# QEDProtocol/city-rollup

Hardware: AMD Instinct MI355X
Metric: ms/NTT at 2^20 Goldilocks (commit-shaped step: 135-column 2^20-row NTT + Poseidon Merkle cap) (lower is better)
Workload: dtype u64 (Goldilocks mod 2^64-2^32+1; the Poseidon MDS layers are evaluated exactly on 32-bit limbs held in f64); 1 GPU; configs[1]: 2^20-row x 135-column trace, forward NTT per column (natural->bit-reversed) + Poseidon Merkle cap height 4; log_n=20, columns=135, cap_height=4

## Files before the change

### city-rollup_amd/cityprover/__init__.py

```python
import ctypes
import os

import numpy as np

from . import build as _build

P = 0xFFFFFFFF00000001
NTT_INVERSE, NTT_BITREV_OUT, NTT_COSET, NTT_BITREV_IN = 1, 2, 4, 8

_u64p = ctypes.POINTER(ctypes.c_uint64)
_vp = ctypes.c_void_p

ABI = {
    "cp_abi_version": (ctypes.c_int, []),
    "cp_device_count": (ctypes.c_int, []),
    "cp_fault_inject": (ctypes.c_int, [ctypes.c_int, ctypes.c_long]),
    "cp_ctx_create": (_vp, [ctypes.c_int]),
    "cp_ctx_destroy": (None, [_vp]),
    "cp_ctx_set_lanes": (ctypes.c_int, [_vp, ctypes.c_int]),
    "cp_ctx_set_device_transcript": (ctypes.c_int, [_vp, ctypes.c_int]),
    "cp_ctx_set_option": (ctypes.c_int, [_vp, ctypes.c_char_p, ctypes.c_long]),
    "cp_last_error": (ctypes.c_char_p, [_vp]),
    "cp_dev_alloc": (ctypes.c_int, [_vp, ctypes.c_size_t, ctypes.POINTER(_vp)]),
    "cp_dev_free": (ctypes.c_int, [_vp, _vp]),
    "cp_host_alloc": (ctypes.c_int, [_vp, ctypes.c_size_t, ctypes.POINTER(_vp)]),
    "cp_host_free": (ctypes.c_int, [_vp, _vp]),
    "cp_h2d": (ctypes.c_int, [_vp, _vp, _vp, ctypes.c_size_t]),
    "cp_d2h": (ctypes.c_int, [_vp, _vp, _vp, ctypes.c_size_t]),
    "cp_d2d": (ctypes.c_int, [_vp, _vp, _vp, ctypes.c_size_t]),
    "cp_sync": (ctypes.c_int, [_vp]),
    "cp_event_create": (ctypes.c_int, [_vp, ctypes.POINTER(_vp)]),
    "cp_event_destroy": (ctypes.c_int, [_vp, _vp]),
    "cp_event_record": (ctypes.c_int, [_vp, _vp]),
    "cp_event_elapsed_ms": (ctypes.c_int, [_vp, _vp, _vp, ctypes.POINTER(ctypes.c_float)]),
    "cp_profile_begin": (ctypes.c_int, [_vp]),
    "cp_profile_end": (ctypes.c_int, [_vp, ctypes.c_char_p, ctypes.c_size_t]),
    "cp_ntt_dev": (ctypes.c_int, [_vp, _vp, ctypes.c_int, ctypes.c_size_t, ctypes.c_size_t,
                                  ctypes.c_uint, ctypes.c_uint64]),
    "cp_ntt": (ctypes.c_int, [_vp, _u64p, ctypes.c_int, ctypes.c_size_t, ctypes.c_uint,
                              ctypes.c_uint64]),
    "cp_lde_dev": (ctypes.c_int, [_vp, _vp, ctypes.c_size_t, ctypes.c_int, ctypes.c_int,
                                  ctypes.c_size_t, ctypes.c_uint64, ctypes.c_uint, _vp,
                                  ctypes.c_size_t]),
    "cp_poseidon_permute_dev": (ctypes.c_int, [_vp, _vp, ctypes.c_size_t]),
    "cp_field_mul": (ctypes.c_int, [_vp, _u64p, _u64p, _u64p, ctypes.c_size_t]),
    "cp_field_mul2": (ctypes.c_int, [_vp, _u64p, _u64p, _u64p, _u64p, _u64p, _u64p, ctypes.c_size_t]),
    "cp_poseidon_permute": (ctypes.c_int, [_vp, _u64p, ctypes.c_size_t]),
    "cp_hash_no_pad": (ctypes.c_int, [_vp, _u64p, ctypes.c_size_t, ctypes.c_size_t, _u64p]),
    "cp_two_to_one": (ctypes.c_int, [_vp, _u64p, _u64p, ctypes.c_size_t, _u64p]),
    "cp_merkle_cols_dev": (ctypes.c_int, [_vp, _vp, ctypes.c_size_t, ctypes.c_size_t,
                                          ctypes.c_size_t, ctypes.c_int, _vp, _vp]),
    "cp_merkle_cap": (ctypes.c_int, [_vp, _u64p, ctypes.c_size_t, ctypes.c_size_t, ctypes.c_int,
                                     _u64p]),
    "cp_commit_dev": (ctypes.c_int, [_vp, _vp, ctypes.c_size_t, ctypes.c_int, ctypes.c_int,
                                     ctypes.c_int, _vp, _vp, _vp, _vp]),
    "cp_commit_batch_dev": (ctypes.c_int, [_vp, _vp, ctypes.c_size_t, ctypes.c_size_t, ctypes.c_int,
                                           ctypes.c_int, ctypes.c_int, _vp, _vp, _vp, _vp]),
}


class CityProverError(RuntimeError):
    pass


_lib = None


def load_library(build_if_missing=True):
    global _lib
    if _lib is not None:
        return _lib
    so = _build.SO
    if not os.path.exists(so):
        if not build_if_missing:
            raise CityProverError(f"{so} not built; run __graft_entry__.build()")
        _build.build()
    lib = ctypes.CDLL(so)
    for name, (res, args) in ABI.items():
        f = getattr(lib, name)
# ... 166 lines not shown
        self._check(self.lib.cp_ntt(self.ctx, _ptr(a), log_n, batch, flags, shift))
        return a

    def intt(self, a, flags=0, shift=0):
        return self.ntt(a, flags | NTT_INVERSE, shift)

    def lde(self, coeffs, rate_bits, shift=7, bitrev=False):
        c = _as_u64(coeffs)
        c2 = c.reshape(1, -1) if c.ndim == 1 else c
        k, n = c2.shape
        log_n = int(n).bit_length() - 1
        din, dout = self.to_device(c2), self.alloc(k * (n << rate_bits))
        try:
            self.lde_dev(din.ptr, log_n, rate_bits, k, dout.ptr, shift, NTT_BITREV_OUT if bitrev else 0)
            out = dout.download().reshape(k, n << rate_bits)
        finally:
            din.free()
            dout.free()
        return out[0] if c.ndim == 1 else out

    def field_mul(self, a, b):
        x, y = _as_u64(a).ravel().copy(), _as_u64(b).ravel().copy()
        assert x.size == y.size
        out = np.zeros(x.size, np.uint64)
        self._check(self.lib.cp_field_mul(self.ctx, _ptr(x), _ptr(y), _ptr(out), x.size))
        return out

    def field_mul2(self, a, b, c, d):
        v = [_as_u64(x).ravel().copy() for x in (a, b, c, d)]
        assert all(x.size == v[0].size for x in v)
        out_ab, out_cd = np.zeros(v[0].size, np.uint64), np.zeros(v[0].size, np.uint64)
        self._check(self.lib.cp_field_mul2(self.ctx, _ptr(v[0]), _ptr(v[1]), _ptr(v[2]), _ptr(v[3]), _ptr(out_ab), _ptr(out_cd), v[0].size))
        return out_ab, out_cd

    def poseidon_permute(self, states):
        s = _as_u64(states).copy()
        assert s.size % 12 == 0
        self._check(self.lib.cp_poseidon_permute(self.ctx, _ptr(s), s.size // 12))
        return s

    def hash_no_pad(self, inputs):
        x = _as_u64(inputs)
        x2 = x.reshape(1, -1) if x.ndim == 1 else x
        out = np.zeros((x2.shape[0], 4), np.uint64)
        self._check(self.lib.cp_hash_no_pad(self.ctx, _ptr(x2), x2.shape[0], x2.shape[1], _ptr(out)))
        return out[0] if x.ndim == 1 else out

    def two_to_one(self, left, right):
        l, r = _as_u64(left), _as_u64(right)
        l2, r2 = l.reshape(-1, 4), r.reshape(-1, 4)
        out = np.zeros_like(l2)
        self._check(self.lib.cp_two_to_one(self.ctx, _ptr(l2), _ptr(r2), l2.shape[0], _ptr(out)))
        return out.reshape(l.shape)

    def merkle_cap(self, rows, cap_height):
        rows = _as_u64(rows)
        n, k = rows.shape
        cap = np.zeros((1 << cap_height, 4), np.uint64)
        self._check(self.lib.cp_merkle_cap(self.ctx, _ptr(rows), n, k, cap_height, _ptr(cap)))
        return cap

    def merkle_cols(self, cols, cap_height, want_digests=False):
        cols = _as_u64(cols)
        k, n = cols.shape
        dc, dcap = self.to_device(cols), self.alloc(4 << cap_height)
        nd = 2 * n - (2 << cap_height)
# ... 1455 lines not shown
```

### city-rollup_amd/csrc/cityprover.hip

```cpp
#include "core.h"
#include "merkle.h"
#include "ntt.h"
#include "ntt16.h"
#include "poseidon.h"
#include "poseidon_coop.h"

namespace {

int get_pow_table(cp_ctx *ctx, uint64_t base, const uint64_t **out) {
  auto it = ctx->pow_tables.find(base);
  if (it != ctx->pow_tables.end()) {
    *out = it->second.get<uint64_t>();
    return CP_OK;
  }
  std::vector<uint64_t> h(3 * ntt::PT_SIZE);
  uint64_t b = base;
  for (int lvl = 0; lvl < 3; lvl++) {
    uint64_t acc = 1;
    for (int j = 0; j < ntt::PT_SIZE; j++) {
      h[lvl * ntt::PT_SIZE + j] = acc;
      acc = gl::mul(acc, b);
    }
    b = acc;
  }
// ... 700 lines not shown
  return cp_d2h(ctx, out_host, o, bytes);
} CP_CATCH(ctx)

__global__ __launch_bounds__(256) void k_field_mul2(const uint64_t *__restrict__ a, const uint64_t *__restrict__ b,
                                                    const uint64_t *__restrict__ c, const uint64_t *__restrict__ d,
                                                    uint64_t *__restrict__ out_ab, uint64_t *__restrict__ out_cd, size_t n) {
  const size_t i = (size_t)blockIdx.x * 256 + threadIdx.x;
  if (i < n) {
    uint64_t r0, r1;
    gl::mul_lazy2(a[i], b[i], c[i], d[i], r0, r1);
    out_ab[i] = gl::canon(r0);
    out_cd[i] = gl::canon(r1);
  }
}

int cp_field_mul2(cp_ctx *ctx, const uint64_t *a_host, const uint64_t *b_host, const uint64_t *c_host, const uint64_t *d_host,
                  uint64_t *out_ab_host, uint64_t *out_cd_host, size_t count) try {
  CHECK_CTX(ctx);
  if (count == 0) return CP_OK;
  if (!a_host || !b_host || !c_host || !d_host || !out_ab_host || !out_cd_host) return set_error(ctx, CP_ERR_INVALID_ARG, "NULL pointer");
  if (count > ((size_t)1 << 27)) return set_error(ctx, CP_ERR_INVALID_ARG, "count too large");
  const size_t bytes = count * sizeof(uint64_t);
  CP_TRY(ensure_scratch(ctx, 6 * bytes));
  uint64_t *a = ctx->scratch.get<uint64_t>(), *b = a + count, *c = b + count, *d = c + count, *o0 = d + count, *o1 = o0 + count;
  CP_TRY(cp_h2d(ctx, a, a_host, bytes));
  CP_TRY(cp_h2d(ctx, b, b_host, bytes));
  CP_TRY(cp_h2d(ctx, c, c_host, bytes));
  CP_TRY(cp_h2d(ctx, d, d_host, bytes));
  LAUNCH(ctx, "field_mul2", k_field_mul2, dim3(blocks_for(count, 256)), dim3(256), a, b, c, d, o0, o1, count);
  CP_TRY(cp_d2h(ctx, out_ab_host, o0, bytes));
  return cp_d2h(ctx, out_cd_host, o1, bytes);
} CP_CATCH(ctx)


int cp_poseidon_permute_dev(cp_ctx *ctx, uint64_t *states, size_t count) try {
  CHECK_CTX(ctx);
  if (count == 0) return CP_OK;
  if (!states) return set_error(ctx, CP_ERR_INVALID_ARG, "states is NULL");
  LAUNCH(ctx, "poseidon_permute", merkle::k_permute, dim3(blocks_for(count, merkle::THREADS)),
         dim3(merkle::THREADS), states, count);
  return CP_OK;
} CP_CATCH(ctx)

int cp_poseidon_permute(cp_ctx *ctx, uint64_t *states_host, size_t count) try {
  CHECK_CTX(ctx);
  if (count == 0) return CP_OK;
  if (!states_host) return set_error(ctx, CP_ERR_INVALID_ARG, "states is NULL");
  size_t bytes = count * 12 * sizeof(uint64_t);
  CP_TRY(ensure_scratch(ctx, bytes));
  CP_TRY(cp_h2d(ctx, ctx->scratch.get(), states_host, bytes));
  CP_TRY(cp_poseidon_permute_dev(ctx, ctx->scratch.get<uint64_t>(), count));
  return cp_d2h(ctx, states_host, ctx->scratch.get(), bytes);
} CP_CATCH(ctx)

int cp_hash_no_pad(cp_ctx *ctx, const uint64_t *in_host, size_t count, size_t len,
                   uint64_t *digests_host) try {
  CHECK_CTX(ctx);
  if (count == 0) return CP_OK;
  if (!digests_host || (!in_host && len)) return set_error(ctx, CP_ERR_INVALID_ARG, "NULL pointer");
  if (len > (1u << 30)) return set_error(ctx, CP_ERR_INVALID_ARG, "len too large");
  size_t in_bytes = count * len * sizeof(uint64_t), out_bytes = count * 32;
  size_t in_al = (in_bytes + 255) & ~(size_t)255;
  CP_TRY(ensure_scratch(ctx, in_al + out_bytes));
  uint64_t *din = ctx->scratch.get<uint64_t>(), *dout = (uint64_t *)(ctx->scratch.get<char>() + in_al);
  if (in_bytes) CP_TRY(cp_h2d(ctx, din, in_host, in_bytes));
  LAUNCH(ctx, "leaf_hash_rows", merkle::k_leaf_hash_rows, dim3(blocks_for(count, merkle::THREADS)),
// ... 111 lines not shown
```

### city-rollup_amd/csrc/gl.h

```cpp
#pragma once
#include <hip/hip_runtime.h>
#include <stdint.h>

#define GL_HD __host__ __device__ __forceinline__
#if defined(__HIP_DEVICE_COMPILE__) && !defined(GL_PORTABLE)
#define GL_DEVICE_ASM 1
#else
#define GL_DEVICE_ASM 0
#endif

namespace gl {

constexpr uint64_t P = 0xFFFFFFFF00000001ULL;
constexpr uint64_t EPS = 0xFFFFFFFFULL;

GL_HD uint64_t canon(uint64_t x) { return x + (x >= P ? EPS : 0); }

GL_HD uint32_t lo32(uint64_t x) { return (uint32_t)x; }
GL_HD uint32_t hi32(uint64_t x) { return (uint32_t)(x >> 32); }
GL_HD uint64_t pack(uint32_t lo, uint32_t hi) { return ((uint64_t)hi << 32) | lo; }

typedef unsigned __int128 u128;

GL_HD uint64_t sub(uint64_t a, uint64_t b) {
// ... 131 lines not shown
  asm("s_nop 1\n\t"
      "v_subb_co_u32_e64 %0, %4, %7, %8, %10\n\t"
      "v_subb_co_u32_e64 %2, %5, %11, %12, %14\n\t"
      "s_nop 0\n\t"
      "v_subbrev_co_u32_e64 %1, %4, 0, %9, %4\n\t"
      "v_subbrev_co_u32_e64 %3, %5, 0, %13, %5\n\t"
      "s_or_b64 %6, %4, %5"
      : "=&v"(tlA), "=&v"(thA), "=&v"(tlB), "=&v"(thB), "=&s"(bA), "=&s"(bB), "=&s"(bm)
      : "v"(lo32(loA)), "v"(hi32(hiA)), "v"(hi32(loA)), "s"(cyA), "v"(lo32(loB)), "v"(hi32(hiB)), "v"(hi32(loB)), "s"(cyB)
      : "scc");
  uint64_t tA = pack(tlA, thA), tB = pack(tlB, thB);
  if (__builtin_expect(bm != 0, 0)) {
    uint32_t nA, nB;
    asm volatile("s_nop 1\n\tv_cndmask_b32 %0, 0, -1, %2\n\tv_cndmask_b32 %1, 0, -1, %3" : "=&v"(nA), "=v"(nB) : "s"(bA), "s"(bB));
    tA -= nA;
    tB -= nB;
  }
  uint64_t fA, fB, cA, cB, cD;
  uint32_t mA, nB;
  asm("v_mad_u64_u32 %0, %1, %8, -1, %9\n\t"
      "v_mad_u64_u32 %3, %4, %10, -1, %11\n\t"
      "s_nop 0\n\t"
      "v_cndmask_b32 %2, 0, -1, %1\n\t"
      "v_cndmask_b32 %5, 0, 1, %4\n\t"
      "v_mad_u64_u32 %6, %7, %5, -1, %3"
      : "=&v"(fA), "=&s"(cA), "=&v"(mA), "=&v"(fB), "=&s"(cB), "=&v"(nB), "=&v"(r1), "=&s"(cD)
      : "v"(lo32(hiA)), "v"(tA), "v"(lo32(hiB)), "v"(tB));
  r0 = fA + mA;
#else
  r0 = mul_lazy(a0, b0);
  r1 = mul_lazy(a1, b1);
#endif
}
GL_HD uint64_t mul(uint64_t a, uint64_t b) {
  uint64_t lo, hi;
  carry_t cy;
  mul_wide_cy(a, b, lo, hi, cy);
  return reduce128(lo, hi, cy);
}
GL_HD uint64_t sqr(uint64_t a) { return mul(a, a); }
GL_HD uint64_t mul_add_lazy(uint64_t a, uint64_t b, uint64_t c) {
  uint64_t lo, hi;
  carry_t cy;
  mul_wide_cy(a, b, lo, hi, cy);
  lo += c;
  hi += lo < c;
  return reduce128_lazy(lo, hi, cy);
}

GL_HD uint64_t pow7(uint64_t x) {
  uint64_t x2 = sqr(x), x4 = sqr(x2), x3 = mul(x, x2);
  return mul(x3, x4);
}

GL_HD uint64_t pow(uint64_t b, uint64_t e) {
  uint64_t r = 1;
  while (e) {
    if (e & 1) r = mul(r, b);
    b = sqr(b);
    e >>= 1;
  }
  return r;
}
GL_HD uint64_t inv(uint64_t a) { return pow(a, P - 2); }

struct Ext {
// ... 12 lines not shown
```

### city-rollup_amd/csrc/ntt16.h

```cpp
#pragma once
#include <type_traits>

#include "gl.h"
#include "ntt.h"

namespace ntt16 {

template <int K>
GL_HD uint64_t mul_pow2(uint64_t x) {
  static_assert(K >= 0 && K < 96, "shift out of range");
  if constexpr (K == 0) {
    return x;
  } else if constexpr (K < 64) {
    return gl::reduce128(x << K, x >> (64 - K));
  } else {
    constexpr int J = K - 64;
    uint64_t y0 = J ? (x << J) : x;
    uint64_t y1 = J ? (x >> (64 - J)) : 0;
    uint64_t t = gl::reduce128(0, y0);
    return gl::sub(t, y1 << 32);
  }
}

template <bool INV, int E>
GL_HD uint64_t diff_times_w16(uint64_t u, uint64_t v) {
  constexpr int SH = ((INV ? 36 : 156) * (E & 15)) % 192;
  constexpr bool NEG = SH >= 96;
  constexpr int K = SH % 96;
  uint64_t d = NEG ? gl::sub(v, u) : gl::sub(u, v);
  return mul_pow2<K>(d);
}

template <bool INV, int B, bool UNIT_T>
GL_HD void stage(uint64_t (&x)[16], uint64_t T) {
#pragma unroll
  for (int m = 0; m < 16; m++) {
    if (m & (1 << B)) continue;
    const int i = m & ((1 << B) - 1);
    uint64_t u = x[m], v = x[m + (1 << B)];
    x[m] = gl::add(u, v);
    uint64_t d;
    switch (i << (3 - B)) {
      case 0: d = diff_times_w16<INV, 0>(u, v); break;
      case 1: d = diff_times_w16<INV, 1>(u, v); break;
      case 2: d = diff_times_w16<INV, 2>(u, v); break;
      case 3: d = diff_times_w16<INV, 3>(u, v); break;
      case 4: d = diff_times_w16<INV, 4>(u, v); break;
      case 5: d = diff_times_w16<INV, 5>(u, v); break;
      case 6: d = diff_times_w16<INV, 6>(u, v); break;
      default: d = diff_times_w16<INV, 7>(u, v); break;
    }
    x[m + (1 << B)] = UNIT_T ? d : gl::mul(d, T);
  }
}

template <bool INV, int NSTAGES, bool UNIT_T>
GL_HD void round16(uint64_t (&x)[16], uint64_t T3) {
#if defined(NTT16_STAGE_TWIDDLES)
  uint64_t T2 = UNIT_T ? 1 : gl::sqr(T3);
  stage<INV, 3, UNIT_T>(x, T3);
  if constexpr (NSTAGES >= 2) {
    stage<INV, 2, UNIT_T>(x, T2);
  }
  if constexpr (NSTAGES >= 3) {
    uint64_t T1 = UNIT_T ? 1 : gl::sqr(T2);
    stage<INV, 1, UNIT_T>(x, T1);
    if constexpr (NSTAGES >= 4) {
      uint64_t T0 = UNIT_T ? 1 : gl::sqr(T1);
      stage<INV, 0, UNIT_T>(x, T0);
    }
  }
#else
  stage<INV, 3, true>(x, 1);
  if constexpr (NSTAGES >= 2) stage<INV, 2, true>(x, 1);
  if constexpr (NSTAGES >= 3) stage<INV, 1, true>(x, 1);
  if constexpr (NSTAGES >= 4) stage<INV, 0, true>(x, 1);
  if constexpr (!UNIT_T) {
    uint64_t pw = T3;
#pragma unroll
    for (int e = 1; e < (1 << NSTAGES); e++) {
      if (e > 1) pw = gl::mul_lazy(pw, T3);
#pragma unroll
      for (int m = 0; m < 16; m++) {
        int em = 0;
        for (int B = 3; B >= 4 - NSTAGES; B--) em += ((m >> B) & 1) << (3 - B);
        if (em == e) x[m] = gl::mul(x[m], pw);
      }
    }
  }
#endif
}

constexpr int LOG_TILE = 12;
constexpr int THREADS = 1 << (LOG_TILE - 4);

__device__ __forceinline__ int pad(int p) { return p + (p >> 4); }

template <bool HALF, typename T>
__device__ __forceinline__ void exchange(T *tile, uint64_t (&x)[16], int Pw, int Fw, int Pr, int Fr) {
  T *w = tile + pad(Pw), *r = tile + pad(Pr);
  if constexpr (HALF) {
    uint32_t lo[16];
#pragma unroll
    for (int m = 0; m < 16; m++) w[pad(m << Fw)] = gl::lo32(x[m]);
// ... 16 lines not shown
}

template <int L, int C, bool ROWS>
__device__ __forceinline__ size_t gidx(int pos, uint32_t tile_id, int q) {
  if (ROWS) return ((size_t)tile_id << LOG_TILE) + pos;
  uint32_t r = pos >> C, o = (tile_id << C) + (pos & ((1 << C) - 1));
  return ((size_t)(o >> q) << (q + L)) | ((size_t)r << q) | (o & ((1u << q) - 1));
}

#ifndef NTT16_MIN_WAVES
#define NTT16_MIN_WAVES 5
#endif
template <int L, int C, bool ROWS, bool INV, bool HALF>
__global__ __launch_bounds__(THREADS, (HALF && !(L == 4 && !ROWS)) ? NTT16_MIN_WAVES : 1) void k_dif_pass16(ntt::PassArgs a) {
  static_assert(L + C == LOG_TILE && L >= 4, "tile shape");
  using tile_t = typename std::conditional<HALF, uint32_t, uint64_t>::type;
  __shared__ tile_t tile[(1 << LOG_TILE) + (1 << (LOG_TILE - 4))];
  constexpr int B0 = ((L - 1) % 4) + 1;
  constexpr int NROUNDS = 1 + (L - B0) / 4;
  const int t = threadIdx.x;
  const int q = a.q;
  uint64_t *poly = a.data + (size_t)blockIdx.y * a.stride + (size_t)blockIdx.z * a.block_stride;
  const uint64_t *in = (a.first && a.src) ? a.src + (size_t)blockIdx.y * a.src_stride : poly;
  const uint64_t *ptab =
      (a.first && a.ptab) ? a.ptab + ((size_t)ntt::bitrev(blockIdx.z, a.block_bits) << a.log_n) : nullptr;
  uint64_t x[16];

  {
    constexpr int f = L - 4;
    constexpr int F = ROWS ? f : C + f;
    const int P = ((t >> F) << (F + 4)) | (t & ((1 << F) - 1));
    const uint64_t *in_t = ROWS ? in + ((size_t)blockIdx.x << LOG_TILE) : in;
    const uint64_t *ptab_t = (ROWS && ptab) ? ptab + ((size_t)blockIdx.x << LOG_TILE) : ptab;
#pragma unroll
    for (int m = 0; m < 16; m++) {
      const size_t idx = gidx<L, C, ROWS>(P + (m << F), blockIdx.x, q);
      uint64_t v = ROWS ? in_t[P + (m << F)] : in[idx];
      if (ptab) v = gl::mul(v, ROWS ? ptab_t[P + (m << F)] : ptab[idx]);
      else if (a.coset_pre && a.first) v = gl::mul(v, ntt::pow_table(a.stab, idx));
      x[m] = v;
    }
    if constexpr (f == 0) {
      round16<INV, B0, true>(x, 1);
    } else {
      const int r = ROWS ? (P & ((1 << L) - 1)) : (P >> C);
      const uint32_t r_lo = r & ((1 << f) - 1);
      uint64_t T3 = ntt::pow_table(a.wtab, (uint64_t)r_lo << (a.log_n - f - 4));
      round16<INV, B0, false>(x, T3);
    }
  }
  constexpr int Flast = ROWS ? 0 : C;
  constexpr int F0 = ROWS ? (L - 4) : C + (L - 4);
  int Plast = ((t >> F0) << (F0 + 4)) | (t & ((1 << F0) - 1));
  int Fprev = F0;
#pragma unroll
  for (int k = 1; k < NROUNDS; k++) {
    const int f = L - B0 - 4 * k;
    const int F = ROWS ? f : C + f;
    const int P = ((t >> F) << (F + 4)) | (t & ((1 << F) - 1));
    exchange<HALF>(tile, x, Plast, Fprev, P, F);
    if (f == 0) {
      round16<INV, 4, true>(x, 1);
    } else {
      const int r = ROWS ? (P & ((1 << L) - 1)) : (P >> C);
      const uint32_t r_lo = r & ((1 << f) - 1);
      uint64_t T3 = ntt::pow_table(a.wtab, (uint64_t)r_lo << (a.log_n - f - 4));
      round16<INV, 4, false>(x, T3);
    }
    Plast = P;
    Fprev = F;
  }
  {
    const int P = Plast;
    if (!ROWS && q > 0) {
      const uint32_t cc = P & ((1 << C) - 1);
      const uint32_t r_base = P >> C;
      const uint32_t o = (blockIdx.x << C) + cc;
      const uint32_t lo = o & ((1u << q) - 1);
      if (lo) {
        const int sh = a.log_n - q - L;
        uint64_t W0 = ntt::pow_table(a.wtab, ((uint64_t)lo * ntt::bitrev(r_base, L)) << sh);
        uint64_t G = ntt::pow_table(a.wtab, ((uint64_t)lo << (L - 4)) << sh);
        uint64_t w = W0;
#pragma unroll
        for (int j = 0; j < 16; j++) {
          const int m = ((j & 1) << 3) | ((j & 2) << 1) | ((j & 4) >> 1) | ((j & 8) >> 3);
          x[m] = gl::mul(x[m], w);
          if (j < 15) w = gl::mul_lazy(w, G);
        }
      }
    }
    if (a.last && a.scale) {
#pragma unroll
      for (int m = 0; m < 16; m++) x[m] = gl::mul(x[m], a.scale);
    }
    if (ROWS && a.natural_out) {
      __syncthreads();
      if constexpr (HALF) {
        uint32_t lo[16];
#pragma unroll
        for (int m = 0; m < 16; m++) tile[pad((int)ntt::bitrev((uint32_t)(P + m), L))] = gl::lo32(x[m]);
        __syncthreads();
#pragma unroll
        for (int m = 0; m < 16; m++) lo[m] = tile[pad(t + (m << (LOG_TILE - 4)))];
        __syncthreads();
#pragma unroll
        for (int m = 0; m < 16; m++) tile[pad((int)ntt::bitrev((uint32_t)(P + m), L))] = gl::hi32(x[m]);
        __syncthreads();
#pragma unroll
        for (int m = 0; m < 16; m++) {
          int pos = t + (m << (LOG_TILE - 4));
          poly[((size_t)blockIdx.x << LOG_TILE) + pos] = gl::pack(lo[m], tile[pad(pos)]);
        }
      } else {
#pragma unroll
        for (int m = 0; m < 16; m++) tile[pad((int)ntt::bitrev((uint32_t)(P + m), L))] = x[m];
        __syncthreads();
#pragma unroll
        for (int m = 0; m < 16; m++) {
          int pos = t + (m << (LOG_TILE - 4));
          poly[((size_t)blockIdx.x << LOG_TILE) + pos] = tile[pad(pos)];
        }
      }
      return;
    }
    if (ROWS && a.staged_store) {
      uint64_t *out_t = poly + ((size_t)blockIdx.x << LOG_TILE);
// ... 50 lines not shown
```

### include/cityprover.h

```cpp
#ifndef CITYPROVER_H
#define CITYPROVER_H

#include <stddef.h>
#include <stdint.h>

#ifdef __cplusplus
extern "C" {
#endif

#define CP_ABI_VERSION 4

typedef enum cp_status {
  CP_OK = 0,
  CP_ERR_INVALID_ARG = -1,
  CP_ERR_NO_DEVICE = -2,
  CP_ERR_HIP = -3,
  CP_ERR_OOM = -4,
  CP_ERR_UNSUPPORTED = -5,
  CP_ERR_INTERNAL = -6,
  CP_ERR_VERIFY = -7
} cp_status;

typedef struct cp_ctx cp_ctx;

// ... 10 lines not shown

int cp_dev_alloc(cp_ctx *ctx, size_t bytes, void **out);
int cp_dev_free(cp_ctx *ctx, void *ptr);
int cp_host_alloc(cp_ctx *ctx, size_t bytes, void **out);
int cp_host_free(cp_ctx *ctx, void *ptr);
int cp_h2d(cp_ctx *ctx, void *dst_dev, const void *src_host, size_t bytes);
int cp_d2h(cp_ctx *ctx, void *dst_host, const void *src_dev, size_t bytes);
int cp_d2d(cp_ctx *ctx, void *dst_dev, const void *src_dev, size_t bytes);
int cp_sync(cp_ctx *ctx);
int cp_event_create(cp_ctx *ctx, void **event_out);
int cp_event_destroy(cp_ctx *ctx, void *event);
int cp_event_record(cp_ctx *ctx, void *event);
int cp_event_elapsed_ms(cp_ctx *ctx, void *start, void *stop, float *ms_out);

int cp_profile_begin(cp_ctx *ctx);
int cp_profile_end(cp_ctx *ctx, char *json_out, size_t cap);

#define CP_NTT_INVERSE 1u
#define CP_NTT_BITREV_OUT 2u
#define CP_NTT_COSET 4u
#define CP_NTT_BITREV_IN 8u
int cp_ntt_dev(cp_ctx *ctx, uint64_t *data_dev, int log_n, size_t batch, size_t stride,
               unsigned flags, uint64_t coset_shift);
int cp_ntt(cp_ctx *ctx, uint64_t *data_host, int log_n, size_t batch, unsigned flags,
           uint64_t coset_shift);

int cp_lde_dev(cp_ctx *ctx, const uint64_t *coeffs_dev, size_t in_stride, int log_n, int rate_bits,
               size_t batch, uint64_t coset_shift, unsigned flags, uint64_t *out_dev,
               size_t out_stride);

int cp_field_mul(cp_ctx *ctx, const uint64_t *a_host, const uint64_t *b_host, uint64_t *out_host, size_t count);
int cp_field_mul2(cp_ctx *ctx, const uint64_t *a_host, const uint64_t *b_host, const uint64_t *c_host, const uint64_t *d_host,
                  uint64_t *out_ab_host, uint64_t *out_cd_host, size_t count);

int cp_poseidon_permute_dev(cp_ctx *ctx, uint64_t *states_dev, size_t count);
int cp_poseidon_permute(cp_ctx *ctx, uint64_t *states_host, size_t count);
int cp_hash_no_pad(cp_ctx *ctx, const uint64_t *in_host, size_t count, size_t len,
                   uint64_t *digests_host);
int cp_two_to_one(cp_ctx *ctx, const uint64_t *left_host, const uint64_t *right_host, size_t count,
                  uint64_t *out_host);

int cp_merkle_cols_dev(cp_ctx *ctx, const uint64_t *cols_dev, size_t n_leaves, size_t leaf_len,
                       size_t col_stride, int cap_height, uint64_t *digests_dev,
                       uint64_t *cap_dev);
int cp_merkle_cap(cp_ctx *ctx, const uint64_t *rows_host, size_t n_leaves, size_t leaf_len,
                  int cap_height, uint64_t *cap_host);

int cp_commit_dev(cp_ctx *ctx, const uint64_t *values_dev, size_t k, int log_n, int rate_bits,
                  int cap_height, uint64_t *coeffs_dev, uint64_t *lde_dev, uint64_t *digests_dev,
                  uint64_t *cap_dev);

int cp_commit_batch_dev(cp_ctx *ctx, const uint64_t *values_dev, size_t k, size_t n_trees, int log_n,
                        int rate_bits, int cap_height, uint64_t *coeffs_dev, uint64_t *lde_dev,
                        uint64_t *digests_dev, uint64_t *caps_dev);

typedef struct cp_shape {
  int degree_bits, num_constants, num_routed_wires, num_wires, num_challenges, num_partial_products,
      quotient_degree_factor;
  int rate_bits, cap_height, pow_bits, num_query_rounds;
  int n_arity;
  int arity_bits[8];
  int zero_knowledge;
  int num_public_inputs;
} cp_shape;
#define CP_SALT_SIZE 4

// ... 377 lines not shown
```

### rust/cityprover-sys/src/ffi.rs

```rust
#![allow(non_camel_case_types, dead_code)]
use std::os::raw::{c_char, c_int, c_long, c_uint, c_void};

pub const CP_ABI_VERSION: c_int = 4;
pub const CP_NTT_INVERSE: c_uint = 1;
pub const CP_NTT_BITREV_OUT: c_uint = 2;
pub const CP_NTT_COSET: c_uint = 4;
pub const CP_NTT_BITREV_IN: c_uint = 8;
pub const CP_SALT_SIZE: usize = 4;
pub const CP_BATCH_FROM_COEFFS: c_uint = 1;
pub const CP_STARK_BATCH_MAX: usize = 64;
pub const CP_PATHS_AUTO: c_uint = 0;
pub const CP_PATHS_LANE: c_uint = 1;
pub const CP_PATHS_COOP: c_uint = 2;
pub const CP_G1_AFFINE_BYTES: usize = 112;
pub const CP_G2_AFFINE_BYTES: usize = 224;
pub const CP_R1CS_NO_TERM_CLASSES: c_uint = 1;
pub const CP_GT_WORDS: usize = 72;
pub const CP_PAIRING_TRUSTED: c_uint = 1;
pub const CP_GROTH16_KEY_FILE_VERSION: usize = 1;
pub const CP_GROTH16_KEY_FILE_RAW: c_uint = 1;
pub const CP_GROTH16_KEY_LOAD_CHECK_TORSION: c_uint = 1;
pub const CP_OK: c_int = 0;
pub const CP_ERR_INVALID_ARG: c_int = -1;
pub const CP_ERR_NO_DEVICE: c_int = -2;
// ... 276 lines not shown
    pub file_bytes: usize,
    pub checksum: u64,
}

extern "C" {
    pub fn cp_abi_version() -> c_int;
    pub fn cp_device_count() -> c_int;
    pub fn cp_ctx_create(device: c_int) -> *mut CpCtx;
    pub fn cp_ctx_destroy(ctx: *mut CpCtx);
    pub fn cp_ctx_set_lanes(ctx: *mut CpCtx, lanes: c_int) -> c_int;
    pub fn cp_ctx_set_device_transcript(ctx: *mut CpCtx, mode: c_int) -> c_int;
    pub fn cp_ctx_set_option(ctx: *mut CpCtx, name: *const c_char, value: c_long) -> c_int;
    pub fn cp_last_error(ctx: *mut CpCtx) -> *const c_char;
    pub fn cp_fault_inject(kind: c_int, after: c_long) -> c_int;
    pub fn cp_dev_alloc(ctx: *mut CpCtx, bytes: usize, out: *mut *mut c_void) -> c_int;
    pub fn cp_dev_free(ctx: *mut CpCtx, ptr: *mut c_void) -> c_int;
    pub fn cp_host_alloc(ctx: *mut CpCtx, bytes: usize, out: *mut *mut c_void) -> c_int;
    pub fn cp_host_free(ctx: *mut CpCtx, ptr: *mut c_void) -> c_int;
    pub fn cp_h2d(ctx: *mut CpCtx, dst_dev: *mut c_void, src_host: *const c_void, bytes: usize) -> c_int;
    pub fn cp_d2h(ctx: *mut CpCtx, dst_host: *mut c_void, src_dev: *const c_void, bytes: usize) -> c_int;
    pub fn cp_d2d(ctx: *mut CpCtx, dst_dev: *mut c_void, src_dev: *const c_void, bytes: usize) -> c_int;
    pub fn cp_sync(ctx: *mut CpCtx) -> c_int;
    pub fn cp_event_create(ctx: *mut CpCtx, event_out: *mut *mut c_void) -> c_int;
    pub fn cp_event_destroy(ctx: *mut CpCtx, event: *mut c_void) -> c_int;
    pub fn cp_event_record(ctx: *mut CpCtx, event: *mut c_void) -> c_int;
    pub fn cp_event_elapsed_ms(ctx: *mut CpCtx, start: *mut c_void, stop: *mut c_void, ms_out: *mut f32) -> c_int;
    pub fn cp_profile_begin(ctx: *mut CpCtx) -> c_int;
    pub fn cp_profile_end(ctx: *mut CpCtx, json_out: *mut c_char, cap: usize) -> c_int;
    pub fn cp_ntt_dev(ctx: *mut CpCtx, data_dev: *mut u64, log_n: c_int, batch: usize, stride: usize, flags: c_uint, coset_shift: u64) -> c_int;
    pub fn cp_ntt(ctx: *mut CpCtx, data_host: *mut u64, log_n: c_int, batch: usize, flags: c_uint, coset_shift: u64) -> c_int;
    pub fn cp_lde_dev(ctx: *mut CpCtx, coeffs_dev: *const u64, in_stride: usize, log_n: c_int, rate_bits: c_int, batch: usize, coset_shift: u64, flags: c_uint, out_dev: *mut u64, out_stride: usize) -> c_int;
    pub fn cp_field_mul(ctx: *mut CpCtx, a_host: *const u64, b_host: *const u64, out_host: *mut u64, count: usize) -> c_int;
    pub fn cp_field_mul2(ctx: *mut CpCtx, a_host: *const u64, b_host: *const u64, c_host: *const u64, d_host: *const u64, out_ab_host: *mut u64, out_cd_host: *mut u64, count: usize) -> c_int;
    pub fn cp_poseidon_permute_dev(ctx: *mut CpCtx, states_dev: *mut u64, count: usize) -> c_int;
    pub fn cp_poseidon_permute(ctx: *mut CpCtx, states_host: *mut u64, count: usize) -> c_int;
    pub fn cp_hash_no_pad(ctx: *mut CpCtx, in_host: *const u64, count: usize, len: usize, digests_host: *mut u64) -> c_int;
    pub fn cp_two_to_one(ctx: *mut CpCtx, left_host: *const u64, right_host: *const u64, count: usize, out_host: *mut u64) -> c_int;
    pub fn cp_merkle_cols_dev(ctx: *mut CpCtx, cols_dev: *const u64, n_leaves: usize, leaf_len: usize, col_stride: usize, cap_height: c_int, digests_dev: *mut u64, cap_dev: *mut u64) -> c_int;
    pub fn cp_merkle_cap(ctx: *mut CpCtx, rows_host: *const u64, n_leaves: usize, leaf_len: usize, cap_height: c_int, cap_host: *mut u64) -> c_int;
    pub fn cp_commit_dev(ctx: *mut CpCtx, values_dev: *const u64, k: usize, log_n: c_int, rate_bits: c_int, cap_height: c_int, coeffs_dev: *mut u64, lde_dev: *mut u64, digests_dev: *mut u64, cap_dev: *mut u64) -> c_int;
    pub fn cp_commit_batch_dev(ctx: *mut CpCtx, values_dev: *const u64, k: usize, n_trees: usize, log_n: c_int, rate_bits: c_int, cap_height: c_int, coeffs_dev: *mut u64, lde_dev: *mut u64, digests_dev: *mut u64, caps_dev: *mut u64) -> c_int;
    pub fn cp_circuit_load(ctx: *mut CpCtx, shape: *const CpShape, circuit_digest: *const u64, cs_values_host: *const u64, k_is_host: *const u64) -> *mut CpCircuit;
    pub fn cp_zs_partial_products_dev(ctx: *mut CpCtx, n_proofs: usize, circuits: *const *mut CpCircuit, wires_values_dev: *const u64, betas_host: *const u64, gammas_host: *const u64, out_dev: *mut u64) -> c_int;
    pub fn cp_circuit_destroy(circuit: *mut CpCircuit);
    pub fn cp_circuit_load_file(ctx: *mut CpCtx, path: *const c_char) -> *mut CpCircuit;
    pub fn cp_circuit_save_file(circuit: *mut CpCircuit, path: *const c_char) -> c_int;
    pub fn cp_circuit_file_info(path: *const c_char, shape_out: *mut CpShape, digest_out: *mut u64, n_gates_out: *mut usize, num_selectors_out: *mut c_int, flags_out: *mut c_uint) -> c_int;
    pub fn cp_circuit_set_public_input_targets(circuit: *mut CpCircuit, row_wire_pairs: *const u32, n_targets: usize) -> c_int;
    pub fn cp_circuit_public_inputs_from_wires(circuit: *mut CpCircuit, wires_values_host: *const u64, public_inputs_out: *mut u64) -> c_int;
    pub fn cp_circuit_shape(circuit: *mut CpCircuit, shape_out: *mut CpShape, digest_out: *mut u64) -> c_int;
    pub fn cp_circuits_batch_compatible(a: *const CpCircuit, b: *const CpCircuit) -> c_int;
    pub fn cp_circuit_cs_cap(circuit: *mut CpCircuit, cap_out_host: *mut u64) -> c_int;
    pub fn cp_prove_tail(circuit: *mut CpCircuit, public_inputs_host: *const u64, n_public_inputs: usize, wires_values_dev: *const u64, zs_pp_values_dev: *const u64, quotient_coeffs_dev: *const u64, use_pow_override: c_int, pow_override: u64, proof_out: *mut *mut u8, proof_len: *mut usize) -> c_int;
    pub fn cp_prove_tail_batch(ctx: *mut CpCtx, n_proofs: usize, circuits: *const *mut CpCircuit, public_inputs_host: *const *const u64, n_public_inputs: *const usize, wires_values_dev: *const u64, zs_pp_values_dev: *const u64, quotient_coeffs_dev: *const u64, use_pow_override: *const c_int, pow_override: *const u64, proofs_out: *mut *mut u8, proof_lens: *mut usize) -> c_int;
    pub fn cp_circuit_set_gates(circuit: *mut CpCircuit, gates: *const CpGate, n_gates: usize, num_selectors: c_int) -> c_int;
    pub fn cp_prove_batch(ctx: *mut CpCtx, n_proofs: usize, circuits: *const *mut CpCircuit, public_inputs_host: *const *const u64, n_public_inputs: *const usize, wires_values_dev: *const u64, use_pow_override: *const c_int, pow_override: *const u64, proofs_out: *mut *mut u8, proof_lens: *mut usize) -> c_int;
    pub fn cp_prove_batch_host(ctx: *mut CpCtx, n_proofs: usize, circuits: *const *mut CpCircuit, public_inputs_host: *const *const u64, n_public_inputs: *const usize, wires_values_host: *const *const u64, use_pow_override: *const c_int, pow_override: *const u64, proofs_out: *mut *mut u8, proof_lens: *mut usize) -> c_int;
    pub fn cp_prove(circuit: *mut CpCircuit, wires_values_host: *const u64, public_inputs_host: *const u64, n_public_inputs: usize, use_pow_override: c_int, pow_override: u64, proof_out: *mut *mut u8, proof_len: *mut usize) -> c_int;
    pub fn cp_prove_batch_zk_host(ctx: *mut CpCtx, n_proofs: usize, circuits: *const *mut CpCircuit, public_inputs_host: *const *const u64, n_public_inputs: *const usize, wires_values_host: *const *const u64, salts_host: *const *const u64, use_pow_override: *const c_int, pow_override: *const u64, proofs_out: *mut *mut u8, proof_lens: *mut usize) -> c_int;
    pub fn cp_batcher_create(ctx: *mut CpCtx, max_batch: usize, linger_us: c_uint) -> *mut CpBatcher;
    pub fn cp_batcher_prove(batcher: *mut CpBatcher, circuit: *mut CpCircuit, wires_values_host: *const u64, public_inputs_host: *const u64, n_public_inputs: usize, use_pow_override: c_int, pow_override: u64, proof_out: *mut *mut u8, proof_len: *mut usize) -> c_int;
    pub fn cp_batcher_get_stats(batcher: *mut CpBatcher, out: *mut CpBatcherStats) -> c_int;
    pub fn cp_batcher_destroy(batcher: *mut CpBatcher);
    pub fn cp_verify(circuit: *mut CpCircuit, proof: *const u8, proof_len: usize) -> c_int;
    pub fn cp_free(ptr: *mut c_void);
    pub fn cp_verify_fri_queries_with_challenges(shape: *const CpShape, proof: *const u8, proof_len: usize, alpha: *const u64, zeta: *const u64, fri_betas: *const u64, x_indices: *const u64) -> c_int;
// ... 70 lines not shown
```

Measured before the change: 0.05007 ms/NTT.

## Pair independent Goldilocks reductions and multiplies in radix-16 NTT rounds

Adds a dual-lane 128-bit Goldilocks reduction in inline GCN assembly and uses it, with the existing paired multiply, throughout the radix-16 NTT kernel: power-of-two twiddle shifts are grouped by form and reduced two at a time, twiddle walks interleave the next-power multiply with the data multiply, and loads, coset pre-multiplies and final scaling are processed in pairs. The goal is to raise instruction-level parallelism and hide carry and VALU latency in the butterfly arithmetic. A test entry point for the paired reduction is exposed through C, Python and Rust. The hand-written assembly with s_nop hazard padding and the larger register footprint could reduce occupancy or introduce correctness risks.

Result: faster. 0.04868 ms/NTT, median of 6 (-2.8%).

```diff
diff --git a/city-rollup_amd/cityprover/__init__.py b/city-rollup_amd/cityprover/__init__.py
--- a/city-rollup_amd/cityprover/__init__.py
+++ b/city-rollup_amd/cityprover/__init__.py
@@ -45,6 +45,7 @@
     "cp_poseidon_permute_dev": (ctypes.c_int, [_vp, _vp, ctypes.c_size_t]),
     "cp_field_mul": (ctypes.c_int, [_vp, _u64p, _u64p, _u64p, ctypes.c_size_t]),
     "cp_field_mul2": (ctypes.c_int, [_vp, _u64p, _u64p, _u64p, _u64p, _u64p, _u64p, ctypes.c_size_t]),
+    "cp_field_reduce2": (ctypes.c_int, [_vp, _u64p, _u64p, _u64p, _u64p, _u64p, _u64p, ctypes.c_size_t]),
     "cp_poseidon_permute": (ctypes.c_int, [_vp, _u64p, ctypes.c_size_t]),
     "cp_hash_no_pad": (ctypes.c_int, [_vp, _u64p, ctypes.c_size_t, ctypes.c_size_t, _u64p]),
     "cp_two_to_one": (ctypes.c_int, [_vp, _u64p, _u64p, ctypes.c_size_t, _u64p]),
@@ -277,6 +278,13 @@
         out_ab, out_cd = np.zeros(v[0].size, np.uint64), np.zeros(v[0].size, np.uint64)
         self._check(self.lib.cp_field_mul2(self.ctx, _ptr(v[0]), _ptr(v[1]), _ptr(v[2]), _ptr(v[3]), _ptr(out_ab), _ptr(out_cd), v[0].size))
         return out_ab, out_cd
+
+    def field_reduce2(self, lo_a, hi_a, lo_b, hi_b):
+        v = [_as_u64(x).ravel().copy() for x in (lo_a, hi_a, lo_b, hi_b)]
+        assert all(x.size == v[0].size for x in v)
+        out_a, out_b = np.zeros(v[0].size, np.uint64), np.zeros(v[0].size, np.uint64)
+        self._check(self.lib.cp_field_reduce2(self.ctx, _ptr(v[0]), _ptr(v[1]), _ptr(v[2]), _ptr(v[3]), _ptr(out_a), _ptr(out_b), v[0].size))
+        return out_a, out_b
 
     def poseidon_permute(self, states):
         s = _as_u64(states).copy()
diff --git a/city-rollup_amd/csrc/cityprover.hip b/city-rollup_amd/csrc/cityprover.hip
--- a/city-rollup_amd/csrc/cityprover.hip
+++ b/city-rollup_amd/csrc/cityprover.hip
@@ -756,6 +756,36 @@
   return cp_d2h(ctx, out_cd_host, o1, bytes);
 } CP_CATCH(ctx)
 
+__global__ __launch_bounds__(256) void k_field_reduce2(const uint64_t *__restrict__ lo_a, const uint64_t *__restrict__ hi_a,
+                                                       const uint64_t *__restrict__ lo_b, const uint64_t *__restrict__ hi_b,
+                                                       uint64_t *__restrict__ out_a, uint64_t *__restrict__ out_b, size_t n) {
+  const size_t i = (size_t)blockIdx.x * 256 + threadIdx.x;
+  if (i < n) {
+    uint64_t r0, r1;
+    gl::reduce128_lazy2(lo_a[i], hi_a[i], lo_b[i], hi_b[i], r0, r1);
+    out_a[i] = gl::canon(r0);
+    out_b[i] = gl::canon(r1);
+  }
+}
+
+int cp_field_reduce2(cp_ctx *ctx, const uint64_t *lo_a_host, const uint64_t *hi_a_host, const uint64_t *lo_b_host, const uint64_t *hi_b_host,
+                     uint64_t *out_a_host, uint64_t *out_b_host, size_t count) try {
+  CHECK_CTX(ctx);
+  if (count == 0) return CP_OK;
+  if (!lo_a_host || !hi_a_host || !lo_b_host || !hi_b_host || !out_a_host || !out_b_host) return set_error(ctx, CP_ERR_INVALID_ARG, "NULL pointer");
+  if (count > ((size_t)1 << 27)) return set_error(ctx, CP_ERR_INVALID_ARG, "count too large");
+  const size_t bytes = count * sizeof(uint64_t);
+  CP_TRY(ensure_scratch(ctx, 6 * bytes));
+  uint64_t *la = ctx->scratch.get<uint64_t>(), *ha = la + count, *lb = ha + count, *hb = lb + count, *o0 = hb + count, *o1 = o0 + count;
+  CP_TRY(cp_h2d(ctx, la, lo_a_host, bytes));
+  CP_TRY(cp_h2d(ctx, ha, hi_a_host, bytes));
+  CP_TRY(cp_h2d(ctx, lb, lo_b_host, bytes));
+  CP_TRY(cp_h2d(ctx, hb, hi_b_host, bytes));
+  LAUNCH(ctx, "field_reduce2", k_field_reduce2, dim3(blocks_for(count, 256)), dim3(256), la, ha, lb, hb, o0, o1, count);
+  CP_TRY(cp_d2h(ctx, out_a_host, o0, bytes));
+  return cp_d2h(ctx, out_b_host, o1, bytes);
+} CP_CATCH(ctx)
+
 
 int cp_poseidon_permute_dev(cp_ctx *ctx, uint64_t *states, size_t count) try {
   CHECK_CTX(ctx);
diff --git a/city-rollup_amd/csrc/gl.h b/city-rollup_amd/csrc/gl.h
--- a/city-rollup_amd/csrc/gl.h
+++ b/city-rollup_amd/csrc/gl.h
@@ -187,6 +187,54 @@
   r1 = mul_lazy(a1, b1);
 #endif
 }
+GL_HD void reduce128_lazy2(uint64_t lo0, uint64_t hi0, uint64_t lo1, uint64_t hi1, uint64_t &r0, uint64_t &r1) {
+#if GL_DEVICE_ASM
+  uint32_t tlA, thA, tlB, thB;
+  uint64_t bA, bB, bm;
+  asm("v_sub_co_u32_e64 %0, %4, %7, %8\n\t"
+      "v_sub_co_u32_e64 %2, %5, %10, %11\n\t"
+      "s_nop 0\n\t"
+      "v_subbrev_co_u32_e64 %1, %4, 0, %9, %4\n\t"
+      "v_subbrev_co_u32_e64 %3, %5, 0, %12, %5\n\t"
+      "s_or_b64 %6, %4, %5"
+      : "=&v"(tlA), "=&v"(thA), "=&v"(tlB), "=&v"(thB), "=&s"(bA), "=&s"(bB), "=&s"(bm)
+      : "v"(lo32(lo0)), "v"(hi32(hi0)), "v"(hi32(lo0)), "v"(lo32(lo1)), "v"(hi32(hi1)), "v"(hi32(lo1))
+      : "scc");
+  uint64_t tA = pack(tlA, thA), tB = pack(tlB, thB);
+  if (__builtin_expect(bm != 0, 0)) {
+    uint32_t nA, nB;
+    asm volatile("s_nop 1\n\tv_cndmask_b32 %0, 0, -1, %2\n\tv_cndmask_b32 %1, 0, -1, %3" : "=&v"(nA), "=v"(nB) : "s"(bA), "s"(bB));
+    tA -= nA;
+    tB -= nB;
+  }
+  uint64_t fA, fB, cA, cB, cD;
+  uint32_t mA, nB;
+  asm("v_mad_u64_u32 %0, %1, %8, -1, %9\n\t"
+      "v_mad_u64_u32 %3, %4, %10, -1, %11\n\t"
+      "s_nop 0\n\t"
+      "v_cndmask_b32 %2, 0, -1, %1\n\t"
+      "v_cndmask_b32 %5, 0, 1, %4\n\t"
+      "v_mad_u64_u32 %6, %7, %5, -1, %3"
+      : "=&v"(fA), "=&s"(cA), "=&v"(mA), "=&v"(fB), "=&s"(cB), "=&v"(nB), "=&v"(r1), "=&s"(cD)
+      : "v"(lo32(hi0)), "v"(tA), "v"(lo32(hi1)), "v"(tB));
+  r0 = fA + mA;
+#else
+  r0 = reduce128_lazy(lo0, hi0);
+  r1 = reduce128_lazy(lo1, hi1);
+#endif
+}
+GL_HD void reduce128_2(uint64_t lo0, uint64_t hi0, uint64_t lo1, uint64_t hi1, uint64_t &r0, uint64_t &r1) {
+  uint64_t t0, t1;
+  reduce128_lazy2(lo0, hi0, lo1, hi1, t0, t1);
+  r0 = canon(t0);
+  r1 = canon(t1);
+}
+GL_HD void mul2(uint64_t a0, uint64_t b0, uint64_t a1, uint64_t b1, uint64_t &r0, uint64_t &r1) {
+  uint64_t t0, t1;
+  mul_lazy2(a0, b0, a1, b1, t0, t1);
+  r0 = canon(t0);
+  r1 = canon(t1);
+}
 GL_HD uint64_t mul(uint64_t a, uint64_t b) {
   uint64_t lo, hi;
   carry_t cy;
diff --git a/city-rollup_amd/csrc/ntt16.h b/city-rollup_amd/csrc/ntt16.h
--- a/city-rollup_amd/csrc/ntt16.h
+++ b/city-rollup_amd/csrc/ntt16.h
@@ -54,6 +54,122 @@
   }
 }
 
+#if defined(NTT16_SINGLE_CHAINS) || defined(NTT16_STAGE_TWIDDLES)
+#define NTT16_PAIRS 0
+#else
+#define NTT16_PAIRS 1
+#endif
+
+template <int K0, int K1>
+GL_HD void mul_pow2_2(uint64_t &x, uint64_t &y) {
+  static_assert(K0 > 0 && K0 < 96 && K1 > 0 && K1 < 96 && (K0 < 64) == (K1 < 64), "two shifts of one form");
+  if constexpr (K0 < 64) {
+    gl::reduce128_2(x << K0, x >> (64 - K0), y << K1, y >> (64 - K1), x, y);
+  } else {
+    constexpr int J0 = K0 - 64, J1 = K1 - 64;
+    const uint64_t x0 = J0 ? (x << J0) : x, x1 = J0 ? (x >> (64 - J0)) : 0;
+    const uint64_t y0 = J1 ? (y << J1) : y, y1 = J1 ? (y >> (64 - J1)) : 0;
+    uint64_t t, u;
+    gl::reduce128_2(0, x0, 0, y0, t, u);
+    x = gl::sub(t, x1 << 32);
+    y = gl::sub(u, y1 << 32);
+  }
+}
+
+template <bool INV>
+constexpr int w16_shift(int E) { return ((INV ? 36 : 156) * (E & 15)) % 192; }
+
+struct ShiftPlan {
+  int a[8], b[8], n;
+};
+template <bool INV, int B>
+constexpr ShiftPlan shift_plan() {
+  ShiftPlan p{};
+  int pend[2] = {-1, -1};
+  for (int m = 0; m < 16; m++) {
+    if (m & (1 << B)) continue;
+    const int K = w16_shift<INV>((m & ((1 << B) - 1)) << (3 - B)) % 96;
+    if (K == 0) continue;
+    const int form = K >= 64, reg = m + (1 << B);
+    if (pend[form] < 0) {
+      pend[form] = reg;
+    } else {
+      p.a[p.n] = pend[form];
+      p.b[p.n++] = reg;
+      pend[form] = -1;
+    }
+  }
+  for (int form = 0; form < 2; form++)
+    if (pend[form] >= 0) {
+      p.a[p.n] = pend[form];
+      p.b[p.n++] = -1;
+    }
+  return p;
+}
+template <bool INV, int B>
+constexpr int reg_shift(int reg) { return w16_shift<INV>((reg & ((1 << B) - 1)) << (3 - B)) % 96; }
+
+template <bool INV, int B, int I = 0>
+GL_HD void apply_shifts(uint64_t (&x)[16]) {
+  constexpr ShiftPlan p = shift_plan<INV, B>();
+  if constexpr (I < p.n) {
+    constexpr int ra = p.a[I], rb = p.b[I];
+    if constexpr (rb < 0) x[ra] = mul_pow2<reg_shift<INV, B>(ra)>(x[ra]);
+    else mul_pow2_2<reg_shift<INV, B>(ra), reg_shift<INV, B>(rb)>(x[ra], x[rb]);
+    apply_shifts<INV, B, I + 1>(x);
+  }
+}
+
+template <bool INV, int B>
+GL_HD void stage_pairs(uint64_t (&x)[16]) {
+#pragma unroll
+  for (int m = 0; m < 16; m++) {
+    if (m & (1 << B)) continue;
+    const bool neg = w16_shift<INV>((m & ((1 << B) - 1)) << (3 - B)) >= 96;
+    const uint64_t u = x[m], v = x[m + (1 << B)];
+    x[m] = gl::add(u, v);
+    x[m + (1 << B)] = neg ? gl::sub(v, u) : gl::sub(u, v);
+  }
+  apply_shifts<INV, B>(x);
+}
+
+constexpr int round_exp(int NSTAGES, int m) {
+  int em = 0;
+  for (int B = 3; B >= 4 - NSTAGES; B--) em += ((m >> B) & 1) << (3 - B);
+  return em;
+}
+constexpr int round_reg(int NSTAGES, int E, int K) {
+  for (int m = 0; m < 16; m++)
+    if (round_exp(NSTAGES, m) == E && K-- == 0) return m;
+  return -1;
+}
+template <int NSTAGES, int E, int K>
+GL_HD void apply_power(uint64_t (&x)[16], uint64_t pw) {
+  constexpr int CNT = 16 >> NSTAGES;
+  if constexpr (K + 1 < CNT) {
+    constexpr int m0 = round_reg(NSTAGES, E, K), m1 = round_reg(NSTAGES, E, K + 1);
+    gl::mul2(x[m0], pw, x[m1], pw, x[m0], x[m1]);
+    apply_power<NSTAGES, E, K + 2>(x, pw);
+  } else if constexpr (K < CNT) {
+    constexpr int m0 = round_reg(NSTAGES, E, K);
+    x[m0] = gl::mul(x[m0], pw);
+  }
+}
+template <int NSTAGES, int E = 1>
+GL_HD void walk_powers(uint64_t (&x)[16], uint64_t pw, uint64_t T3) {
+  constexpr int LAST = (1 << NSTAGES) - 1;
+  if constexpr (E < LAST) {
+    constexpr int m0 = round_reg(NSTAGES, E, 0);
+    uint64_t next, r;
+    gl::mul_lazy2(pw, T3, x[m0], pw, next, r);
+    x[m0] = gl::canon(r);
+    apply_power<NSTAGES, E, 1>(x, pw);
+    walk_powers<NSTAGES, E + 1>(x, next, T3);
+  } else {
+    apply_power<NSTAGES, E, 0>(x, pw);
+  }
+}
+
 template <bool INV, int NSTAGES, bool UNIT_T>
 GL_HD void round16(uint64_t (&x)[16], uint64_t T3) {
 #if defined(NTT16_STAGE_TWIDDLES)
@@ -70,6 +186,12 @@
       stage<INV, 0, UNIT_T>(x, T0);
     }
   }
+#elif NTT16_PAIRS
+  stage_pairs<INV, 3>(x);
+  if constexpr (NSTAGES >= 2) stage_pairs<INV, 2>(x);
+  if constexpr (NSTAGES >= 3) stage_pairs<INV, 1>(x);
+  if constexpr (NSTAGES >= 4) stage_pairs<INV, 0>(x);
+  if constexpr (!UNIT_T) walk_powers<NSTAGES>(x, T3, T3);
 #else
   stage<INV, 3, true>(x, 1);
   if constexpr (NSTAGES >= 2) stage<INV, 2, true>(x, 1);
@@ -152,6 +274,7 @@
     const int P = ((t >> F) << (F + 4)) | (t & ((1 << F) - 1));
     const uint64_t *in_t = ROWS ? in + ((size_t)blockIdx.x << LOG_TILE) : in;
     const uint64_t *ptab_t = (ROWS && ptab) ? ptab + ((size_t)blockIdx.x << LOG_TILE) : ptab;
+#if !NTT16_PAIRS
 #pragma unroll
     for (int m = 0; m < 16; m++) {
       const size_t idx = gidx<L, C, ROWS>(P + (m << F), blockIdx.x, q);
@@ -160,6 +283,18 @@
       else if (a.coset_pre && a.first) v = gl::mul(v, ntt::pow_table(a.stab, idx));
       x[m] = v;
     }
+#else
+#pragma unroll
+    for (int m = 0; m < 16; m += 2) {
+      const int p0 = P + (m << F), p1 = P + ((m + 1) << F);
+      const size_t idx0 = gidx<L, C, ROWS>(p0, blockIdx.x, q), idx1 = gidx<L, C, ROWS>(p1, blockIdx.x, q);
+      uint64_t v0 = ROWS ? in_t[p0] : in[idx0], v1 = ROWS ? in_t[p1] : in[idx1];
+      if (ptab) gl::mul2(v0, ROWS ? ptab_t[p0] : ptab[idx0], v1, ROWS ? ptab_t[p1] : ptab[idx1], v0, v1);
+      else if (a.coset_pre && a.first) gl::mul2(v0, ntt::pow_table(a.stab, idx0), v1, ntt::pow_table(a.stab, idx1), v0, v1);
+      x[m] = v0;
+      x[m + 1] = v1;
+    }
+#endif
     if constexpr (f == 0) {
       round16<INV, B0, true>(x, 1);
     } else {
@@ -205,14 +340,30 @@
 #pragma unroll
         for (int j = 0; j < 16; j++) {
           const int m = ((j & 1) << 3) | ((j & 2) << 1) | ((j & 4) >> 1) | ((j & 8) >> 3);
+#if NTT16_PAIRS
+          if (j < 15) {
+            uint64_t r, next;
+            gl::mul_lazy2(x[m], w, w, G, r, next);
+            x[m] = gl::canon(r);
+            w = next;
+          } else {
+            x[m] = gl::mul(x[m], w);
+          }
+#else
           x[m] = gl::mul(x[m], w);
           if (j < 15) w = gl::mul_lazy(w, G);
+#endif
         }
       }
     }
     if (a.last && a.scale) {
+#if NTT16_PAIRS
+#pragma unroll
+      for (int m = 0; m < 16; m += 2) gl::mul2(x[m], a.scale, x[m + 1], a.scale, x[m], x[m + 1]);
+#else
 #pragma unroll
       for (int m = 0; m < 16; m++) x[m] = gl::mul(x[m], a.scale);
+#endif
     }
     if (ROWS && a.natural_out) {
       __syncthreads();
diff --git a/include/cityprover.h b/include/cityprover.h
--- a/include/cityprover.h
+++ b/include/cityprover.h
@@ -66,6 +66,8 @@
 int cp_field_mul(cp_ctx *ctx, const uint64_t *a_host, const uint64_t *b_host, uint64_t *out_host, size_t count);
 int cp_field_mul2(cp_ctx *ctx, const uint64_t *a_host, const uint64_t *b_host, const uint64_t *c_host, const uint64_t *d_host,
                   uint64_t *out_ab_host, uint64_t *out_cd_host, size_t count);
+int cp_field_reduce2(cp_ctx *ctx, const uint64_t *lo_a_host, const uint64_t *hi_a_host, const uint64_t *lo_b_host,
+                     const uint64_t *hi_b_host, uint64_t *out_a_host, uint64_t *out_b_host, size_t count);
 
 int cp_poseidon_permute_dev(cp_ctx *ctx, uint64_t *states_dev, size_t count);
 int cp_poseidon_permute(cp_ctx *ctx, uint64_t *states_host, size_t count);
diff --git a/rust/cityprover-sys/src/ffi.rs b/rust/cityprover-sys/src/ffi.rs
--- a/rust/cityprover-sys/src/ffi.rs
+++ b/rust/cityprover-sys/src/ffi.rs
@@ -332,6 +332,7 @@
     pub fn cp_lde_dev(ctx: *mut CpCtx, coeffs_dev: *const u64, in_stride: usize, log_n: c_int, rate_bits: c_int, batch: usize, coset_shift: u64, flags: c_uint, out_dev: *mut u64, out_stride: usize) -> c_int;
     pub fn cp_field_mul(ctx: *mut CpCtx, a_host: *const u64, b_host: *const u64, out_host: *mut u64, count: usize) -> c_int;
     pub fn cp_field_mul2(ctx: *mut CpCtx, a_host: *const u64, b_host: *const u64, c_host: *const u64, d_host: *const u64, out_ab_host: *mut u64, out_cd_host: *mut u64, count: usize) -> c_int;
+    pub fn cp_field_reduce2(ctx: *mut CpCtx, lo_a_host: *const u64, hi_a_host: *const u64, lo_b_host: *const u64, hi_b_host: *const u64, out_a_host: *mut u64, out_b_host: *mut u64, count: usize) -> c_int;
     pub fn cp_poseidon_permute_dev(ctx: *mut CpCtx, states_dev: *mut u64, count: usize) -> c_int;
     pub fn cp_poseidon_permute(ctx: *mut CpCtx, states_host: *mut u64, count: usize) -> c_int;
     pub fn cp_hash_no_pad(ctx: *mut CpCtx, in_host: *const u64, count: usize, len: usize, digests_host: *mut u64) -> c_int;
```
